# hank-kuo-cs/Volumetric-Primitives-Net

Measured on NVIDIA B200. Metric: primitive-loss fwd+bwd samples/sec, higher is better.
Workload: dtype f32

## Files before the change

### volumetric-primitives-net_b200/csrc/chamfer_tc.cu

```cuda
#include <cuda_fp16.h>
#include "common.cuh"

namespace vpn {

constexpr int kTcBlk = 128;
constexpr int kTcEpiWarps = 16;
constexpr int kTcThreads = (kTcEpiWarps + 4) * 32;
constexpr int kTcBlkBytes = kTcBlk * 32;
constexpr float kTcBig = 1.0e30f;
constexpr int kTcDefaultHunits = 0;

__device__ __forceinline__ uint32_t tc_smem_u32(const void* p) { return (uint32_t)__cvta_generic_to_shared(p); }
__device__ __forceinline__ float tc_inf() { return __int_as_float(0x7f800000); }

__device__ __forceinline__ uint64_t tc_desc(uint32_t saddr) {
  return (uint64_t)((saddr & 0x3FFFF) >> 4) | ((uint64_t)(128 >> 4) << 16) | ((uint64_t)(256 >> 4) << 32) | (1ull << 46);
}
constexpr uint32_t kTcIdesc = (1u << 4) | (0u << 7) | (0u << 10) | ((uint32_t)(2 * kTcBlk >> 3) << 17) | ((uint32_t)(kTcBlk >> 4) << 24);

constexpr uint32_t kTcIdescHalf = (1u << 4) | (0u << 7) | (0u << 10) | ((uint32_t)(kTcBlk >> 3) << 17) | ((uint32_t)(kTcBlk >> 4) << 24);
constexpr uint32_t kTcIdescHalfF16 = (0u << 4) | (0u << 7) | (0u << 10) | ((uint32_t)(kTcBlk >> 3) << 17) | ((uint32_t)(kTcBlk >> 4) << 24);

__device__ __forceinline__ void tc_mma(uint32_t d_tmem, uint64_t a, uint64_t b, uint32_t accumulate, uint32_t idesc = kTcIdesc) {
#if defined(VPN_TC_VARIANT) && VPN_TC_VARIANT == 3
// ... 85 lines not shown
  if (is_row) { x *= -2.f; y *= -2.f; z *= -2.f; }
  uint32_t hxy, lxy, hzn, lzn;
  tc_split2(x, y, hxy, lxy); tc_split2(z, n2, hzn, lzn);
  const uint32_t ones = 0x3c003c00u;
  uint4 k0, k1;
  if (is_row) {
    k0 = make_uint4(__byte_perm(hxy, hxy, 0x1010), __byte_perm(lxy, lxy, 0x1010), __byte_perm(hxy, hxy, 0x3232), __byte_perm(lxy, lxy, 0x3232));
    k1 = make_uint4(__byte_perm(hzn, hzn, 0x1010), __byte_perm(lzn, lzn, 0x1010), __byte_perm(hzn, lzn, 0x7632), ones);
  } else {
    const uint32_t wx = __byte_perm(hxy, lxy, 0x5410), wy = __byte_perm(hxy, lxy, 0x7632), wz = __byte_perm(hzn, lzn, 0x5410);
    k0 = make_uint4(wx, wx, wy, wy);
    k1 = make_uint4(wz, wz, ones, __byte_perm(hzn, lzn, 0x7632));
  }
  unsigned char* base = tile + (idx >> 3) * 256 + (idx & 7) * 16;
  *reinterpret_cast<uint4*>(base) = k0;
  *reinterpret_cast<uint4*>(base + 128) = k1;
  return n2;
}

struct TcSmem {
  unsigned char* rows; unsigned char* cols; float* rs_best; uint4* rs_mask; float* colw;
  u64* bars; float* red; uint32_t* tmem_slot; uint32_t* skip;
};
constexpr int kTcPlanWords = 128;
constexpr int kTcSkipWords = 128;
__host__ __device__ inline size_t tc_smem_bytes(int NB) {
  return (size_t)NB * kTcBlkBytes + 4 * kTcBlkBytes + 2 * (size_t)NB * kTcBlk * 20 + 2 * 2 * 2 * kTcBlk * 16 + 16 * 8 + 96 * 4 + 16 +
         kTcSkipWords * 4;
}
__device__ __forceinline__ TcSmem tc_carve(unsigned char* p, int NB) {
  TcSmem s;
  s.rows = p; p += (size_t)NB * kTcBlkBytes;
  s.cols = p; p += 4 * kTcBlkBytes;
  s.rs_best = reinterpret_cast<float*>(p); p += 2 * (size_t)NB * kTcBlk * 4;
  s.rs_mask = reinterpret_cast<uint4*>(p); p += 2 * (size_t)NB * kTcBlk * 16;
  s.colw = reinterpret_cast<float*>(p); p += 2 * 2 * 2 * kTcBlk * 16;
  s.bars = reinterpret_cast<u64*>(p); p += 16 * 8;
  s.red = reinterpret_cast<float*>(p); p += 96 * 4;
  s.tmem_slot = reinterpret_cast<uint32_t*>(p); p += 16;
  s.skip = reinterpret_cast<uint32_t*>(p);
  return s;
}

__device__ __forceinline__ float tc_lane_min4x32(uint32_t taddr, uint32_t empty_bar, int lane, float (&u)[4]) {
#if defined(VPN_TC_VARIANT) && VPN_TC_VARIANT == 2
  __syncwarp();
  if (lane == 0) tc_mbar_arrive(empty_bar);
// ... 274 lines not shown
  const float slack_rel = 6.103515625e-05f + 1.0986328125e-03f;
  const float slack_abs = __fmaf_ru(2.5025e-4f, rho2 * (S * S), 1.1930e-06f);
  if (tid == 0 && split == 0) tslack[(size_t)b * ntiles + tile_i] = make_float2(slack_rel, slack_abs * invS2);
  const uint32_t tbase = *sm.tmem_slot;

  const int nc = c_last - c_first;
  const int hc = (nc + 1) >> 1;
  const uint32_t* rawR = sm.skip; const uint32_t* rawC = sm.skip + 64;
  for (int i = tid; i < kTcPlanWords; i += kTcThreads) sm.skip[i] = plan_masks ? plan_masks[(size_t)cta * kTcPlanWords + i] : 0u;
  __syncthreads();
  if (warp == kTcEpiWarps + 2 && stats != nullptr) {
    unsigned s0 = 0, s1 = 0;
    for (int c = lane; c < nc; c += 32) { s0 += __popc(rawR[c] & ((1u << NB) - 1u)); s1 += __popc(rawC[c] & ((1u << NB) - 1u)); }
#pragma unroll
    for (int o = 16; o > 0; o >>= 1) { s0 += __shfl_xor_sync(0xffffffffu, s0, o); s1 += __shfl_xor_sync(0xffffffffu, s1, o); }
    if (lane == 0) {
      atomicAdd(&stats[0], (u64)(2 * nc * NB));
      atomicAdd(&stats[1], (u64)(s0 + s1));
#ifdef VPN_TC_COUNTERS
      atomicAdd(&stats[6], (u64)(nc * NB - s0));
      atomicAdd(&stats[7], (u64)(nc * NB - s1));
#endif
    }
  }
#ifdef VPN_TC_COUNTERS
  long long t_mark = 0;
  if (tid == 0 && stats != nullptr) {
    unsigned livechunks = 0, passes = 0;
    for (int c = 0; c < nc; ++c) livechunks += ((~rawC[c]) & ((1u << NB) - 1u)) ? 1u : 0u;
    for (int cc = 0; cc < 2 * hc; ++cc) passes += tc_pass_needed(cc < hc ? cc : cc - hc, nc, NB, cc < hc ? rawR : rawC) ? 1u : 0u;
    atomicAdd(&stats[8], (u64)livechunks);
    atomicAdd(&stats[9], (u64)passes);
    t_mark = clock64();
    atomicAdd(&stats[2], (u64)(t_mark - t_start));
  }
#define TC_MARK(slot) if (tid == 0 && stats != nullptr) { const long long t_ = clock64(); atomicAdd(&stats[slot], (u64)(t_ - t_mark)); t_mark = t_; }
#else
#define TC_MARK(slot)
#endif
  if (warp >= kTcEpiWarps && warp < kTcEpiWarps + 2) {
    const int g = warp - kTcEpiWarps;
    uint32_t seq = 0;
    float tx[4], ty[4], tz[4];
    const uint32_t nbmask = (1u << NB) - 1u;
    auto next_needed = [&](int cc) { while (cc < 2 * hc && !tc_pass_needed(cc < hc ? cc : cc - hc, nc, NB, cc < hc ? rawR : rawC)) ++cc; return cc; };
    auto half_live = [&](int cc) {
// ... 99 lines not shown
      for (uint32_t live = ~rawR[2 * j + h] & nbmask & (0x55555555u << p); live; live &= live - 1) {
        const int r = __ffs((int)live) - 1;
        tc_mbar_wait(my_full, it & 1);
        tc_fence_after();
        float mu[4];
        const float m = tc_lane_min4x32_h<HUNITS>(tlane, my_empty, lane, mu);
        ++it;
        const int ri = r * kTcBlk + li;
        const float best = my_best[ri];
        if (m <= tc_thr(best, slack_rel, slack_abs)) {
          const float t = tc_thr(fminf(best, m), slack_rel, slack_abs);
          const uint32_t nib = (mu[0] <= t ? 1u : 0u) | (mu[1] <= t ? 2u : 0u) | (mu[2] <= t ? 4u : 0u) | (mu[3] <= t ? 8u : 0u);
          if (tc_thr(m, slack_rel, slack_abs) < best) my_mask[ri] = make_uint4(0u, 0u, 0u, 0u);
          reinterpret_cast<uint32_t*>(my_mask + ri)[j >> 3] |= nib << ((j & 7) * 4);
          if (m < best) my_best[ri] = m;
        }
      }
    }
    TC_MARK(3)
    int cseq = 0;
    float4* xch = reinterpret_cast<float4*>(sm.colw) + (size_t)p * 4 * kTcBlk;
    for (int c = p; c < nc; c += 2) {
      const uint32_t livec = ~rawC[c] & nbmask;
      if (livec == 0u) {
        const int col = (c_first + c) * kTcBlk + li;
        if (h == 0 && col < M) { const size_t o = ((size_t)b * ntiles + tile_i) * M + col; cbest[o] = tc_inf(); cmask[o] = 0ull; }
        continue;
      }
      float best = tc_inf(); u64 mask = 0ull;
      for (uint32_t live = livec & (0x55555555u << h); live; live &= live - 1) {
        const int r = __ffs((int)live) - 1;
        tc_mbar_wait(my_full, it & 1);
        tc_fence_after();
        float mu[4];
        const float m = tc_lane_min4x32_h<HUNITS>(tlane, my_empty, lane, mu);
        ++it;
        if (m <= tc_thr(best, slack_rel, slack_abs)) {
          const float t = tc_thr(fminf(best, m), slack_rel, slack_abs);
          const uint32_t nib = (mu[0] <= t ? 1u : 0u) | (mu[1] <= t ? 2u : 0u) | (mu[2] <= t ? 4u : 0u) | (mu[3] <= t ? 8u : 0u);
          const float tm = tc_thr(m, slack_rel, slack_abs);
          mask = ((tm < best) ? 0ull : mask) | ((u64)nib << (4 * r));
          best = fminf(best, m);
        }
      }
      float4* slot = xch + (size_t)(cseq & 1) * 2 * kTcBlk;
      slot[h * kTcBlk + li] = make_float4(best, __uint_as_float((uint32_t)mask), __uint_as_float((uint32_t)(mask >> 32)), 0.f);
      asm volatile("bar.sync %0, 64;" :: "r"(1 + q + 4 * p) : "memory");
      if ((cseq & 1) == h) {
        const int col = (c_first + c) * kTcBlk + li;
        if (col < M) {
          const float4 other = slot[(h ^ 1) * kTcBlk + li];
// ... 3 lines not shown
          const u64 m2 = ((best <= t) ? mask : 0ull) | ((other.x <= t) ? omask : 0ull);
          const size_t o = ((size_t)b * ntiles + tile_i) * M + col;
          cbest[o] = b2 * invS2; cmask[o] = m2;
        }
      }
      ++cseq;
    }
  }
  TC_MARK(4)
  tc_fence_before();
  __syncthreads();
  if (warp == 0) asm volatile("tcgen05.dealloc.cta_group::1.sync.aligned.b32 %0, 512;" :: "r"(tbase) : "memory");
  const size_t mask_plane = (size_t)gridDim.x / ntiles * P;
  for (int i = tid; i < TM; i += kTcThreads) {
    const int row = tile_i * TM + i;
    if (row < P) {
      const float b0 = sm.rs_best[i], b1 = sm.rs_best[TM + i];
      const float best = fminf(b0, b1);
      const float t = tc_thr(best, slack_rel, slack_abs);
      const uint4 k0 = sm.rs_mask[i], k1 = sm.rs_mask[TM + i];
      const bool in0 = b0 <= t, in1 = b1 <= t;
      const size_t o = ((size_t)b * nsplit + split) * P + row;
      rbest[o] = best * invS2;
      rmask[o] = (in0 ? tc_spread_nibbles(k0.x) : 0ull) | (in1 ? (tc_spread_nibbles(k1.x) << 4) : 0ull);
      rmask[mask_plane + o] = (in0 ? tc_spread_nibbles(k0.y) : 0ull) | (in1 ? (tc_spread_nibbles(k1.y) << 4) : 0ull);
      rmask[2 * mask_plane + o] = (in0 ? tc_spread_nibbles(k0.z) : 0ull) | (in1 ? (tc_spread_nibbles(k1.z) << 4) : 0ull);
      rmask[3 * mask_plane + o] = (in0 ? tc_spread_nibbles(k0.w) : 0ull) | (in1 ? (tc_spread_nibbles(k1.w) << 4) : 0ull);
    }
  }
  TC_MARK(5)
}

__global__ void __launch_bounds__(256)
chamfer_flagged_kernel(const float* __restrict__ p1, const float* __restrict__ p2, float* __restrict__ min1,
                       int* __restrict__ idx1, float* __restrict__ min2, int* __restrict__ idx2,
                       const int* __restrict__ fallback, int P, int M) {
  const int b = blockIdx.y;
  if (fallback[b] == 0) return;
  const float* A = p1 + (size_t)b * P * 3;
  const float* T = p2 + (size_t)b * M * 3;
  for (int dir = 0; dir < 2; ++dir) {
    const float* X = dir ? T : A; const float* Y = dir ? A : T;
    const int nx = dir ? M : P, ny = dir ? P : M;
    float* mn = (dir ? min2 + (size_t)b * M : min1 + (size_t)b * P);
    int* ix = (dir ? idx2 + (size_t)b * M : idx1 + (size_t)b * P);
    for (int i = blockIdx.x * blockDim.x + threadIdx.x; i < nx; i += gridDim.x * blockDim.x) {
      const float x = X[3 * (size_t)i], y = X[3 * (size_t)i + 1], z = X[3 * (size_t)i + 2];
      float bv = tc_inf(); int bj = 0;
      bool nan_seen = false;
      for (int j = 0; j < ny; ++j) {
// ... 9 lines not shown
  }
}

__global__ void __launch_bounds__(256)
chamfer_tc_bounds_kernel(const float* __restrict__ p2, float* __restrict__ tmax, int M) {
  __shared__ float red[8];
  const float* T = p2 + (size_t)blockIdx.x * M * 3;
  float m = 0.f;
  for (int i = threadIdx.x; i < 3 * M; i += 256) {
    const float v = fabsf(T[i]);
    m = (v <= m) ? m : v;
  }
#pragma unroll
  for (int o = 16; o > 0; o >>= 1) { const float x = __shfl_xor_sync(0xffffffffu, m, o); m = (x <= m) ? m : x; }
  if ((threadIdx.x & 31) == 0) red[threadIdx.x >> 5] = m;
  __syncthreads();
  if (threadIdx.x == 0) {
    for (int w = 1; w < 8; ++w) m = (red[w] <= m) ? m : red[w];
    tmax[blockIdx.x] = m;
  }
}

size_t chamfer_tc_smem_bytes(int NB) { return tc_smem_bytes(NB); }
int chamfer_tc_plan_words() { return kTcPlanWords; }


int chamfer_tc_launch(const float* p1, const float* p2, float* rbest, u64* rmask, float* cbest, u64* cmask,
                      float2* tslack, int* fallback, float* tmax, const float* cbox, const float* rbox, const float* rthr,
                      const float* cub, u64* stats, uint32_t* plan_masks, int* plan_work, int* plan_order, int with_bounds,
                      int B, int P, int M, int NB, int ntiles, int nsplit, int nchunks, int cps, cudaStream_t s) {
  static DeviceOnce once;
  const size_t smem = tc_smem_bytes(NB);
  {
    cudaError_t e = set_dyn_smem(chamfer_tc_kernel<0>, (int)tc_smem_bytes(16), once);
    for (int k = 0; k < 4 && e == cudaSuccess; ++k) {
      void (*kern)(const float*, const float*, float*, u64*, float*, u64*, float2*, int*, const float*, const uint32_t*, const int*, u64*,
                   int, int, int, int, int, int, int) = k == 0 ? chamfer_tc_kernel<1> : (k == 1 ? chamfer_tc_kernel<2> : (k == 2 ? chamfer_tc_kernel<3> : chamfer_tc_kernel<4>));
      static DeviceOnce more[4];
      e = set_dyn_smem(kern, (int)tc_smem_bytes(16), more[k]);
    }
    if (e != cudaSuccess) { vpn_set_error("chamfer tc: smem attribute: %s", cudaGetErrorString(e)); return VPN_ERR_CUDA; }
  }
  int rc;
  if (with_bounds) {
    chamfer_tc_bounds_kernel<<<B, 256, 0, s>>>(p2, tmax, M);
    if ((rc = vpn_check_launch("chamfer_tc_bounds_kernel"))) return rc;
  }
// ... 34 lines not shown
```

### volumetric-primitives-net_b200/csrc/chamfer_tiled.cu

```cuda
#include <cstdlib>
#include <mutex>
#include <type_traits>
#include "common.cuh"

namespace vpn {

enum { MODE_EXACT = 0, MODE_DIFF = 1, MODE_EXPAND = 2, MODE_TC = 3 };

constexpr int kTThreads = 256;
constexpr int kTWarps = kTThreads / 32;
constexpr int kCW = 128;
constexpr int kMaxChunksPerSplit = 64;
constexpr float kBig = 1.0e30f;

__device__ __forceinline__ u64 pk(float a, float b) { u64 r; asm("mov.b64 %0, {%1,%2};" : "=l"(r) : "f"(a), "f"(b)); return r; }
__device__ __forceinline__ void upk(u64 v, float& a, float& b) { asm("mov.b64 {%0,%1}, %2;" : "=f"(a), "=f"(b) : "l"(v)); }
__device__ __forceinline__ u64 add2(u64 a, u64 b) { u64 r; asm("add.rn.f32x2 %0, %1, %2;" : "=l"(r) : "l"(a), "l"(b)); return r; }
__device__ __forceinline__ u64 sub2(u64 a, u64 b) { u64 r; asm("sub.rn.f32x2 %0, %1, %2;" : "=l"(r) : "l"(a), "l"(b)); return r; }
__device__ __forceinline__ u64 mul2(u64 a, u64 b) { u64 r; asm("mul.rn.f32x2 %0, %1, %2;" : "=l"(r) : "l"(a), "l"(b)); return r; }
__device__ __forceinline__ u64 fma2(u64 a, u64 b, u64 c) { u64 r; asm("fma.rn.f32x2 %0, %1, %2, %3;" : "=l"(r) : "l"(a), "l"(b), "l"(c)); return r; }
__device__ __forceinline__ float min3f(float a, float b, float c) { float r; asm("min.f32 %0, %1, %2, %3;" : "=f"(r) : "f"(a), "f"(b), "f"(c)); return r; }
__device__ __forceinline__ float warp_min_f32(float a) { float r; asm volatile("redux.sync.min.f32 %0, %1, 0xffffffff;" : "=f"(r) : "f"(a)); return r; }
__device__ __forceinline__ float inf_f() { return __int_as_float(0x7f800000); }

// ... 457 lines not shown
              d[kk] = exact_d2s(rc.x, rc.y, rc.z, q.x, q.y, q.z);
              dm = fminf(dm, d[kk]);
            }
            int at;
            const int st = unit_scan(d, dm, lane, &at);
            if (st == 1) atomicMin(&key[r], ((u64)__float_as_uint(sqrtf(dm)) << 32) | (unsigned)__float_as_int(src[at].w));
            else if (st == 2) { const u64 kv = unit_exact_walk(rc.x, rc.y, rc.z, src, 0, 1); if (kv != ~0ull) atomicMin(&key[r], kv); }
          }
          group_sync(bar);
        }
        if (valid) {
          const u64 kv = key[gt];
          const size_t orow = orow_of();
          min1[orow] = __uint_as_float((unsigned)(kv >> 32));
          idx1[orow] = (int)(unsigned)(kv & 0xffffffffu);
        }
        group_sync(bar);
      }
    }
  }
}

__global__ void chamfer_col_thr_kernel(const float* __restrict__ cbest, const float2* __restrict__ tslack,
                                       float* __restrict__ cthr, int M, int ntiles) {
  const int b = blockIdx.y;
  const int col = blockIdx.x * blockDim.x + threadIdx.x;
  if (col >= M) return;
  float g = inf_f(), rel = 0.f, ab = 0.f;
  for (int ti = 0; ti < ntiles; ++ti) {
    g = fminf(g, cbest[((size_t)b * ntiles + ti) * M + col]);
    const float2 sl = tslack[(size_t)b * ntiles + ti];
    rel = fmaxf(rel, sl.x); ab = fmaxf(ab, sl.y);
  }
  cthr[(size_t)b * M + col] = thr_of(g, rel, ab);
}

template <int R, bool TC, int NT>
__global__ void __launch_bounds__(NT, 1024 / NT)
chamfer_recover_cols_kernel(const float* __restrict__ p1, const float* __restrict__ p2,
                            const float* __restrict__ cbest, const void* __restrict__ cmask_,
                            const float* __restrict__ cthr, u64* __restrict__ key2, int P, int M, int ntiles,
                            const int* __restrict__ skip, const int* __restrict__ rperm) {
  constexpr int TM = TC ? 128 * R : kTThreads * R;
  constexpr int kSub = TC ? 1 : ((R >= 4) ? 4 : R);
  constexpr int kRunsPerSub = TC ? 1 : R / kSub;
  constexpr int kPer = TC ? 4096 / NT : 8;
  constexpr int kBitBits = TC ? 6 : 4;
  using mask_t = typename std::conditional<TC, u64, unsigned>::type;
  const mask_t* __restrict__ cmask = reinterpret_cast<const mask_t*>(cmask_);
  const mask_t kBitMask = TC ? (mask_t)((4 * R >= 64) ? ~0ull : ((1ull << (4 * R)) - 1ull)) : (mask_t)0xffu;
  if (skip && skip[blockIdx.y]) return;
  extern __shared__ __align__(16) unsigned char smem_raw[];
  float4* rows = reinterpret_cast<float4*>(smem_raw);
  __shared__ unsigned items[kItemCap];
  __shared__ int warp_sums[33];
  const int b = blockIdx.y, ti = blockIdx.x, tid = threadIdx.x, lane = tid & 31;
  const float* A = p1 + (size_t)b * P * 3;
  const float qnan = __int_as_float(0x7fc00000);
  for (int i = tid; i < TM; i += NT) {
    int rowi = ti * TM + i;
    rows[i] = rowi < P ? make_float4(A[3 * (size_t)rowi], A[3 * (size_t)rowi + 1], A[3 * (size_t)rowi + 2],
                                     __int_as_float(rperm ? rperm[(size_t)b * P + rowi] : rowi))
                       : make_float4(qnan, qnan, qnan, __int_as_float(0x7fffffff));
  }
  const size_t rec0 = ((size_t)b * ntiles + ti) * M;
  for (int slab = 0; slab < M; slab += NT * kPer) {
    mask_t mk[kPer];
    int cnt = 0;
#pragma unroll
    for (int u = 0; u < kPer; ++u) {
      const int col = slab + u * NT + tid;
      mk[u] = 0;
      if (col < M && cbest[rec0 + col] <= cthr[(size_t)b * M + col]) mk[u] = cmask[rec0 + col] & kBitMask;
      cnt += TC ? __popcll((u64)mk[u]) : __popc((unsigned)mk[u]);
    }
    int total;
    const int off = block_exclusive_scan<NT>(cnt, warp_sums, &total);
    for (int base = 0; base < total; base += kItemCap) {
      int j = off;
#pragma unroll
      for (int u = 0; u < kPer; ++u)
        for (mask_t mm = mk[u]; mm; mm &= mm - 1, ++j)
          if (j >= base && j < base + kItemCap)
            items[j - base] = ((unsigned)(u * NT + tid) << kBitBits) |
                              (unsigned)((TC ? __ffsll((long long)mm) : __ffs((int)mm)) - 1);
      __syncthreads();
      const int units = min(kItemCap, total - base) * kSub;
      for (int it = tid; it < units; it += NT) {
        const unsigned item = items[it / kSub];
        const int col = slab + (int)(item >> kBitBits), w = item & ((1u << kBitBits) - 1u), sub = it % kSub;
        const float* t = p2 + 3 * ((size_t)b * M + col);
        const float tx = __ldg(t), ty = __ldg(t + 1), tz = __ldg(t + 2);
        u64 best = ~0ull;
#pragma unroll 1
        for (int rr = sub * kRunsPerSub; rr < (sub + 1) * kRunsPerSub; ++rr) {
          const int base_row = TC ? (w * 32) : (rr * kTThreads + w * 32);
// ... 13 lines not shown
        }
        if (best != ~0ull) atomicMin(&key2[(size_t)b * M + col], best);
      }
      __syncthreads();
    }
  }
}

__global__ void chamfer_unpack_key_kernel(const u64* __restrict__ key, float* __restrict__ mn, int* __restrict__ idx, size_t n,
                                          const int* __restrict__ skip, int per_sample, const int* __restrict__ perm) {
  size_t i = (size_t)blockIdx.x * blockDim.x + threadIdx.x;
  if (i >= n) return;
  const size_t smp = i / (size_t)per_sample;
  if (skip && skip[smp]) return;
  u64 k = key[i];
  const size_t o = perm ? smp * (size_t)per_sample + (size_t)perm[i] : i;
  mn[o] = __uint_as_float((unsigned)(k >> 32));
  idx[o] = (int)(unsigned)(k & 0xffffffffu);
}

struct TiledPlan { int R, ntiles, nchunks, nsplit, cps, tc, TM; };

size_t chamfer_tc_smem_bytes(int NB);
int chamfer_tc_plan_words();
int chamfer_tc_launch(const float* p1, const float* p2, float* rbest, u64* rmask, float* cbest, u64* cmask,
                      float2* tslack, int* fallback, float* tmax, const float* cbox, const float* rbox, const float* rthr,
                      const float* cub, u64* stats, unsigned* plan_masks, int* plan_work, int* plan_order, int with_bounds,
                      int B, int P, int M, int NB, int ntiles, int nsplit, int nchunks, int cps, cudaStream_t s);
int chamfer_prep_launch(const float* p1, const float* p2, float* p2s, float4* p2v, int* perm, float* cbox, float* rbox, float* rthr,
                        float* cub, float* tmax, float* p1s, int* rperm, unsigned long long* stats, int B, int P, int M, cudaStream_t s);
int chamfer_flagged_launch(const float* p1, const float* p2, float* min1, int* idx1, float* min2, int* idx2,
                           const int* fallback, int B, int P, int M, cudaStream_t s);

static void finish_plan(TiledPlan& pl, int B, long long slots, int min_cps) {
  long long base = (long long)pl.ntiles * B;
  long long s = (4 * slots + base - 1) / base;
  long long smin = (pl.nchunks + kMaxChunksPerSplit - 1) / kMaxChunksPerSplit;
  long long smax = pl.nchunks / min_cps;
  if (s > smax) s = smax;
  if (s < smin) s = smin;
  if (s > pl.nchunks) s = pl.nchunks;
  if (s < 1) s = 1;
  pl.cps = (int)((pl.nchunks + s - 1) / s);
  pl.nsplit = (pl.nchunks + pl.cps - 1) / pl.cps;
}

static bool make_plan(int B, int P, int M, int sm_count, TiledPlan& pl) {
// ... 42 lines not shown
struct TiledWs { size_t rbest, rmask, cbest, cmask, tslack, fallback, tmax, cthr, key2, p2s, p2v, perm, cbox, rbox, rthr, cub, pmask, pwork, porder, p1s, rperm, total; };
static TiledWs ws_layout(int B, int P, int M, const TiledPlan& pl) {
  TiledWs w; size_t o = 0;
  w.rbest = o; o += al256((size_t)B * pl.nsplit * P * 4);
  w.rmask = o; o += al256((size_t)B * pl.nsplit * P * 8 * (pl.tc ? 4 : 1));
  w.cbest = o; o += al256((size_t)B * pl.ntiles * M * 4);
  w.cmask = o; o += al256((size_t)B * pl.ntiles * M * (pl.tc ? 8 : 4));
  w.tslack = o; o += al256((size_t)B * pl.ntiles * 8);
  w.fallback = o; o += al256((size_t)B * 4 + 8 + 128);
  w.tmax = o; o += al256((size_t)B * 4);
  w.cthr = o; o += al256((size_t)B * M * 4);
  w.key2 = o; o += al256((size_t)B * M * 8);
  w.p2s = w.p2v = w.perm = w.cbox = w.rbox = w.rthr = w.cub = w.pmask = w.pwork = w.porder = w.p1s = w.rperm = 0;
  if (pl.tc) {
    const size_t nrb = (size_t)(P + 127) / 128;
    w.p2s = o; o += al256((size_t)B * M * 12);
    w.p2v = o; o += al256((size_t)B * pl.nchunks * kCW * 16);
    w.perm = o; o += al256((size_t)B * M * 4);
    w.cbox = o; o += al256((size_t)B * pl.nchunks * 32);
    w.rbox = o; o += al256((size_t)B * nrb * 32);
    w.rthr = o; o += al256((size_t)B * nrb * 4);
    w.cub = o; o += al256((size_t)B * pl.nchunks * 4);
    const size_t ncta = (size_t)pl.ntiles * pl.nsplit * B;
    w.pmask = o; o += al256(ncta * (size_t)chamfer_tc_plan_words() * 4);
    w.pwork = o; o += al256(ncta * 4);
    w.porder = o; o += al256(ncta * 4);
    w.p1s = o; o += al256((size_t)B * P * 12);
    w.rperm = o; o += al256((size_t)B * P * 4);
  }
  w.total = o;
  return w;
}

static bool plan_for(int mode, int B, int P, int M, TiledPlan& pl) {
  const int kPlanSms = device_sm_count();
  if (mode == MODE_TC) return make_plan_tc(B, P, M, kPlanSms, pl);
  if (mode >= 0) return make_plan(B, P, M, kPlanSms, pl);
  return make_plan_tc(B, P, M, kPlanSms, pl) || make_plan(B, P, M, kPlanSms, pl);
}

int chamfer_tiled_supported(int B, int P, int M, int mode) {
  TiledPlan pl;
  return plan_for(mode, B, P, M, pl) ? 1 : 0;
}

int chamfer_tiled_uses_tc(int B, int P, int M, int mode) {
  TiledPlan pl;
// ... 37 lines not shown
}

template <int R>
static int launch_main_mode(int mode, const float* p1, const float* p2, char* ws, const TiledWs& wl, const TiledPlan& pl,
                            int B, int P, int M, int only_flagged, cudaStream_t s) {
  switch (mode) {
    case MODE_EXACT: return launch_main<R, MODE_EXACT>(p1, p2, ws, wl, pl, B, P, M, only_flagged, s);
    case MODE_DIFF:  return launch_main<R, MODE_DIFF>(p1, p2, ws, wl, pl, B, P, M, only_flagged, s);
    default:         return launch_main<R, MODE_EXPAND>(p1, p2, ws, wl, pl, B, P, M, only_flagged, s);
  }
}

static int launch_any(int mode, const float* p1, const float* p2, char* ws, const TiledWs& wl, const TiledPlan& pl,
                      int B, int P, int M, int only_flagged, cudaStream_t s) {
  switch (pl.R) {
    case 16: return launch_main_mode<16>(mode, p1, p2, ws, wl, pl, B, P, M, only_flagged, s);
    case 8:  return launch_main_mode<8>(mode, p1, p2, ws, wl, pl, B, P, M, only_flagged, s);
    default: return launch_main_mode<4>(mode, p1, p2, ws, wl, pl, B, P, M, only_flagged, s);
  }
}

template <int R, bool TC>
static int launch_recover_cols(const float* p1, const float* p2, const float* cb, const void* cmk, const float* cthr,
                               u64* key2, int B, int P, int M, int ntiles, const int* skip, const int* rperm, cudaStream_t s) {
  static DeviceOnce once, once_half;
  const size_t smem = (size_t)(TC ? 128 * R : kTThreads * R) * sizeof(float4);
  if (TC && (long long)ntiles * B >= 2LL * device_sm_count()) {
    if (set_dyn_smem(chamfer_recover_cols_kernel<R, TC, 512>, (int)smem, once_half) != cudaSuccess) {
      vpn_set_error("chamfer tiled: smem attribute (cols recovery)"); return VPN_ERR_CUDA;
    }
    chamfer_recover_cols_kernel<R, TC, 512><<<dim3(ntiles, B), 512, smem, s>>>(p1, p2, cb, cmk, cthr, key2, P, M, ntiles, skip, rperm);
    return vpn_check_launch("chamfer_recover_cols_kernel");
  }
  if (set_dyn_smem(chamfer_recover_cols_kernel<R, TC, kRecThreads>, (int)smem, once) != cudaSuccess) {
    vpn_set_error("chamfer tiled: smem attribute (cols recovery)"); return VPN_ERR_CUDA;
  }
  chamfer_recover_cols_kernel<R, TC, kRecThreads><<<dim3(ntiles, B), kRecThreads, smem, s>>>(p1, p2, cb, cmk, cthr, key2, P, M, ntiles, skip, rperm);
  return vpn_check_launch("chamfer_recover_cols_kernel");
}

struct SideStream { cudaStream_t s = nullptr; cudaEvent_t fork = nullptr, join = nullptr; bool ok = false; std::mutex mu; };
static SideStream g_side[64];
static SideStream* side_stream_for(cudaStream_t s) {
  int dev = 0;
  if (cudaGetDevice(&dev) != cudaSuccess || dev < 0 || dev >= 64) return nullptr;
  SideStream& ss = g_side[dev];
  if (ss.ok) return &ss;
  cudaStreamCaptureStatus st = cudaStreamCaptureStatusNone;
  if (cudaStreamIsCapturing(s, &st) != cudaSuccess || st != cudaStreamCaptureStatusNone) { cudaGetLastError(); return nullptr; }
  std::lock_guard<std::mutex> lock(ss.mu);
  if (!ss.ok) {
    if (cudaStreamCreateWithFlags(&ss.s, cudaStreamNonBlocking) != cudaSuccess ||
        cudaEventCreateWithFlags(&ss.fork, cudaEventDisableTiming) != cudaSuccess ||
        cudaEventCreateWithFlags(&ss.join, cudaEventDisableTiming) != cudaSuccess) { cudaGetLastError(); return nullptr; }
    ss.ok = true;
  }
  return &ss;
}

int chamfer_tiled_fwd(const float* p1, const float* p2, float* min1, int* idx1, float* min2, int* idx2,
                      int B, int P, int M, void* ws_, size_t ws_bytes, int mode, cudaStream_t s, cudaEvent_t* ev) {
  TiledPlan pl;
  if (!plan_for(mode, B, P, M, pl)) { vpn_set_error("chamfer tiled: unsupported shape"); return VPN_ERR_SHAPE; }
  if (mode < 0) mode = pl.tc ? MODE_TC : MODE_EXPAND;
  TiledWs wl = ws_layout(B, P, M, pl);
  if (ws_bytes < wl.total) { vpn_set_error("chamfer tiled: workspace too small (%zu < %zu)", ws_bytes, wl.total); return VPN_ERR_WORKSPACE; }
  char* ws = reinterpret_cast<char*>(ws_);
  int* fallback = reinterpret_cast<int*>(ws + wl.fallback);
  const int* skip = nullptr;
  int rc;
  if (ev) cudaEventRecord(ev[0], s);
  const size_t flag_bytes = (((size_t)B * 4 + 7) & ~(size_t)7) + 128;
  if (mode == MODE_EXPAND || mode == MODE_TC) {
    if (cudaMemsetAsync(fallback, 0, flag_bytes, s) != cudaSuccess) { vpn_set_error("chamfer tiled: memset failed"); return VPN_ERR_CUDA; }
  }
  const float* p2w = p2;
  const int* perm = nullptr;
  const float4* p2v = nullptr;
  const float* p1w = p1;
  const int* rperm = nullptr;
  if (mode == MODE_TC) {
    float* p2s = reinterpret_cast<float*>(ws + wl.p2s);
    int* pm = reinterpret_cast<int*>(ws + wl.perm);
    float* cbox = reinterpret_cast<float*>(ws + wl.cbox); float* rbox = reinterpret_cast<float*>(ws + wl.rbox);
    float* rthr = reinterpret_cast<float*>(ws + wl.rthr); float* cub = reinterpret_cast<float*>(ws + wl.cub);
    float* tmax = reinterpret_cast<float*>(ws + wl.tmax);
    u64* stats = reinterpret_cast<u64*>(ws + wl.fallback + (((size_t)B * 4 + 7) & ~(size_t)7));
    const bool prune = tuning_value(kTuneTcPrune) != 2;
    if (prune) {
      float4* pv = reinterpret_cast<float4*>(ws + wl.p2v);
      float* p1s = reinterpret_cast<float*>(ws + wl.p1s);
      int* rp = reinterpret_cast<int*>(ws + wl.rperm);
      if ((rc = chamfer_prep_launch(p1, p2, p2s, pv, pm, cbox, rbox, rthr, cub, tmax, p1s, rp, stats, B, P, M, s))) return rc;
      p2w = p2s; perm = pm; p2v = pv; p1w = p1s; rperm = rp;
    }
    rc = chamfer_tc_launch(p1w, p2w, reinterpret_cast<float*>(ws + wl.rbest), reinterpret_cast<u64*>(ws + wl.rmask),
                           reinterpret_cast<float*>(ws + wl.cbest), reinterpret_cast<u64*>(ws + wl.cmask),
                           reinterpret_cast<float2*>(ws + wl.tslack), fallback, tmax, prune ? cbox : nullptr, rbox, rthr, cub, stats,
                           reinterpret_cast<unsigned*>(ws + wl.pmask), reinterpret_cast<int*>(ws + wl.pwork),
                           reinterpret_cast<int*>(ws + wl.porder), prune ? 0 : 1, B, P, M, pl.R, pl.ntiles, pl.nsplit, pl.nchunks,
                           pl.cps, s);
    if (rc) return rc;
    if (ev) cudaEventRecord(ev[1], s);
    if ((rc = chamfer_flagged_launch(p1, p2, min1, idx1, min2, idx2, fallback, B, P, M, s))) return rc;
    skip = fallback;
  } else {
    if ((rc = launch_any(mode, p1, p2, ws, wl, pl, B, P, M, 0, s))) return rc;
    if (ev) cudaEventRecord(ev[1], s);
    if (mode == MODE_EXPAND) {
      if ((rc = launch_any(MODE_DIFF, p1, p2, ws, wl, pl, B, P, M, 1, s))) return rc;
    }
  }
  if (ev) cudaEventRecord(ev[2], s);
  SideStream* side = tuning_value(kTuneSerialRecovery) ? nullptr : side_stream_for(s);
  std::unique_lock<std::mutex> side_lock;
  cudaStream_t sc = s;
  if (side) {
// ... 4 lines not shown
  {
    static DeviceOnce once_rows;
    const size_t smem_rows = kRowsFixedSmem + (size_t)(pl.nchunks < kSegChunks ? pl.nchunks : kSegChunks) * kCW * sizeof(float4);
    if (set_dyn_smem(chamfer_recover_rows_kernel, (int)(kRowsFixedSmem + kSegChunks * kCW * sizeof(float4)), once_rows) != cudaSuccess) {
      vpn_set_error("chamfer tiled: smem attribute (rows recovery)"); return VPN_ERR_CUDA;
    }
    const int nblk = (P + kRowGroup - 1) / kRowGroup;
    const long long nitems = (long long)nblk * B;
    if (nitems > 0x7fffffffLL) { vpn_set_error("chamfer tiled: too many row blocks"); return VPN_ERR_SHAPE; }
    const int sms = device_sm_count();
    chamfer_recover_rows_kernel<<<(unsigned)(nitems < sms ? nitems : sms), kRecThreads, smem_rows, s>>>(
        p1w, p2w, p2v, pl.nchunks * kCW, reinterpret_cast<const float*>(ws + wl.rbest), reinterpret_cast<const u64*>(ws + wl.rmask),
        pl.tc ? 4 : 1, (size_t)B * pl.nsplit * P, reinterpret_cast<const float2*>(ws + wl.tslack), min1, idx1, P, M, pl.nchunks,
        pl.nsplit, pl.cps, pl.TM, pl.ntiles, skip, nblk, (int)nitems, rperm);
    if ((rc = vpn_check_launch("chamfer_recover_rows_kernel"))) return rc;
  }
  if (ev) cudaEventRecord(ev[3], s);
  const float* cb = reinterpret_cast<const float*>(ws + wl.cbest);
  const void* cmk = ws + wl.cmask;
  const float2* tsl = reinterpret_cast<const float2*>(ws + wl.tslack);
  float* cthr = reinterpret_cast<float*>(ws + wl.cthr);
  u64* key2 = reinterpret_cast<u64*>(ws + wl.key2);
  if (cudaMemsetAsync(key2, 0xFF, (size_t)B * M * 8, sc) != cudaSuccess) { vpn_set_error("chamfer tiled: memset failed"); return VPN_ERR_CUDA; }
  chamfer_col_thr_kernel<<<dim3((M + 255) / 256, B), 256, 0, sc>>>(cb, tsl, cthr, M, pl.ntiles);
  if ((rc = vpn_check_launch("chamfer_col_thr_kernel"))) return rc;
  if (pl.tc) {
    switch (pl.R) {
      case 16: rc = launch_recover_cols<16, true>(p1w, p2w, cb, cmk, cthr, key2, B, P, M, pl.ntiles, skip, rperm, sc); break;
      case 8:  rc = launch_recover_cols<8, true>(p1w, p2w, cb, cmk, cthr, key2, B, P, M, pl.ntiles, skip, rperm, sc); break;
      default: rc = launch_recover_cols<4, true>(p1w, p2w, cb, cmk, cthr, key2, B, P, M, pl.ntiles, skip, rperm, sc); break;
    }
  } else {
    switch (pl.R) {
      case 16: rc = launch_recover_cols<16, false>(p1, p2, cb, cmk, cthr, key2, B, P, M, pl.ntiles, skip, nullptr, sc); break;
      case 8:  rc = launch_recover_cols<8, false>(p1, p2, cb, cmk, cthr, key2, B, P, M, pl.ntiles, skip, nullptr, sc); break;
      default: rc = launch_recover_cols<4, false>(p1, p2, cb, cmk, cthr, key2, B, P, M, pl.ntiles, skip, nullptr, sc); break;
    }
  }
  if (rc) return rc;
  {
    size_t n = (size_t)B * M;
    chamfer_unpack_key_kernel<<<(unsigned)((n + 255) / 256), 256, 0, sc>>>(key2, min2, idx2, n, skip, M, perm);
  }
  rc = vpn_check_launch("chamfer_unpack_key_kernel");
  if (side) {
    if (cudaEventRecord(side->join, sc) != cudaSuccess || cudaStreamWaitEvent(s, side->join, 0) != cudaSuccess) {
      vpn_set_error("chamfer tiled: stream join failed"); rc = VPN_ERR_CUDA;
    }
  }
  if (ev) cudaEventRecord(ev[4], s);
  return rc;
}

}
```

### volumetric-primitives-net_b200/csrc/common.cuh

```cuda
#pragma once
#include <cuda_runtime.h>
#include <stdint.h>
#include <atomic>

#define VPN_OK 0
#define VPN_ERR_CUDA (-1)
#define VPN_ERR_SHAPE (-2)
#define VPN_ERR_ARG (-3)
#define VPN_ERR_WORKSPACE (-4)

#define VPN_PI 3.1415927410125732f

void vpn_set_error(const char* fmt, ...);
int vpn_check_launch(const char* what);

namespace vpn {

typedef unsigned long long u64;

struct DeviceOnce { std::atomic<unsigned long long> mask{0}; };
template <typename K>
inline cudaError_t set_dyn_smem(K kernel, int bytes, DeviceOnce& once) {
  int dev = 0;
  cudaError_t e = cudaGetDevice(&dev);
  if (e != cudaSuccess) return e;
  const unsigned long long bit = dev < 64 ? (1ull << dev) : 0ull;
  if (bit && (once.mask.load(std::memory_order_acquire) & bit)) return cudaSuccess;
  e = cudaFuncSetAttribute(kernel, cudaFuncAttributeMaxDynamicSharedMemorySize, bytes);
  if (e == cudaSuccess && bit) once.mask.fetch_or(bit, std::memory_order_release);
  return e;
}
int device_sm_count();
int tuning_value(int key);
enum { kTuneTiledR = 0, kTuneTcNb = 1, kTuneEmdCluster = 2, kTuneTcPrune = 3, kTuneSerialRecovery = 4, kTuneArVariant = 5, kTuneArCtas = 6, kTuneArThreads = 7, kTuneArGridDiv = 8, kTunePrepNearCols = 9, kTunePrepRepsCols = 10, kTunePrepNearRows = 11, kTunePrepRepsRows = 12, kTunePrepProbe = 13, kTunePrepDeterministic = 14, kTuneTcHunits = 15, kTuneCount = 16 };

struct Pose {
  float r[9];
  float qn[4];
  float s, c;
  float len;
};

__device__ __forceinline__ float mod1(float w) {
  float m = fmodf(w, 1.0f);
  if (m != 0.0f && m < 0.0f) m += 1.0f;
  return m;
}

__device__ __forceinline__ void make_pose(const float* __restrict__ q, Pose& p) {
  float a = q[0], b = q[1], cc = q[2], w = q[3];
  float half = __fdiv_rn(__fmul_rn(__fmul_rn(mod1(w), 2.0f), VPN_PI), 2.0f);
  float s = sinf(half), c = cosf(half);
  float ux = a * s, uy = b * s, uz = cc * s, uw = c;
  float len = sqrtf(ux * ux + uy * uy + uz * uz + uw * uw);
  float x = ux / len, y = uy / len, z = uz / len, ww = uw / len;
  p.s = s; p.c = c; p.len = len;
  p.qn[0] = x; p.qn[1] = y; p.qn[2] = z; p.qn[3] = ww;
// ... 53 lines not shown
```

Baseline: 34500.

## Skip writing dead column records and consult prune plan in downstream col kernels

The tensor-core chamfer kernel no longer writes inf/zero sentinel records for fully pruned column chunks. Instead the column-threshold and column-recovery kernels read the prune plan masks and treat those records as dead, so the redundant stores and later reads are avoided. The col-threshold loop is restructured into 32-tile batches with a warp ballot over the plan words. It also adds counter-only diagnostics under a compile flag. The risk is that correctness now depends on the plan indexing in the two consumers matching exactly.

```diff
diff --git a/volumetric-primitives-net_b200/csrc/chamfer_tc.cu b/volumetric-primitives-net_b200/csrc/chamfer_tc.cu
--- a/volumetric-primitives-net_b200/csrc/chamfer_tc.cu
+++ b/volumetric-primitives-net_b200/csrc/chamfer_tc.cu
@@ -131,7 +131,6 @@
   unsigned char* rows; unsigned char* cols; float* rs_best; uint4* rs_mask; float* colw;
   u64* bars; float* red; uint32_t* tmem_slot; uint32_t* skip;
 };
-constexpr int kTcPlanWords = 128;
 constexpr int kTcSkipWords = 128;
 __host__ __device__ inline size_t tc_smem_bytes(int NB) {
   return (size_t)NB * kTcBlkBytes + 4 * kTcBlkBytes + 2 * (size_t)NB * kTcBlk * 20 + 2 * 2 * 2 * kTcBlk * 16 + 16 * 8 + 96 * 4 + 16 +
@@ -452,6 +451,13 @@
       atomicAdd(&stats[7], (u64)(nc * NB - s1));
 #endif
     }
+#ifdef VPN_TC_COUNTERS
+    unsigned sdead = 0;
+    for (int c = lane; c < nc; c += 32) sdead += (rawC[c] & ((1u << NB) - 1u)) == ((1u << NB) - 1u) ? 1u : 0u;
+#pragma unroll
+    for (int o = 16; o > 0; o >>= 1) sdead += __shfl_xor_sync(0xffffffffu, sdead, o);
+    if (lane == 0) atomicAdd(&stats[14], (u64)sdead | ((u64)nc << 32));
+#endif
   }
 #ifdef VPN_TC_COUNTERS
   long long t_mark = 0;
@@ -597,11 +603,7 @@
     float4* xch = reinterpret_cast<float4*>(sm.colw) + (size_t)p * 4 * kTcBlk;
     for (int c = p; c < nc; c += 2) {
       const uint32_t livec = ~rawC[c] & nbmask;
-      if (livec == 0u) {
-        const int col = (c_first + c) * kTcBlk + li;
-        if (h == 0 && col < M) { const size_t o = ((size_t)b * ntiles + tile_i) * M + col; cbest[o] = tc_inf(); cmask[o] = 0ull; }
-        continue;
-      }
+      if (livec == 0u) continue;
       float best = tc_inf(); u64 mask = 0ull;
       for (uint32_t live = livec & (0x55555555u << h); live; live &= live - 1) {
         const int r = __ffs((int)live) - 1;
@@ -651,10 +653,30 @@
       const bool in0 = b0 <= t, in1 = b1 <= t;
       const size_t o = ((size_t)b * nsplit + split) * P + row;
       rbest[o] = best * invS2;
-      rmask[o] = (in0 ? tc_spread_nibbles(k0.x) : 0ull) | (in1 ? (tc_spread_nibbles(k1.x) << 4) : 0ull);
-      rmask[mask_plane + o] = (in0 ? tc_spread_nibbles(k0.y) : 0ull) | (in1 ? (tc_spread_nibbles(k1.y) << 4) : 0ull);
-      rmask[2 * mask_plane + o] = (in0 ? tc_spread_nibbles(k0.z) : 0ull) | (in1 ? (tc_spread_nibbles(k1.z) << 4) : 0ull);
-      rmask[3 * mask_plane + o] = (in0 ? tc_spread_nibbles(k0.w) : 0ull) | (in1 ? (tc_spread_nibbles(k1.w) << 4) : 0ull);
+      const u64 w0 = (in0 ? tc_spread_nibbles(k0.x) : 0ull) | (in1 ? (tc_spread_nibbles(k1.x) << 4) : 0ull);
+      const u64 w1 = (in0 ? tc_spread_nibbles(k0.y) : 0ull) | (in1 ? (tc_spread_nibbles(k1.y) << 4) : 0ull);
+      const u64 w2 = (in0 ? tc_spread_nibbles(k0.z) : 0ull) | (in1 ? (tc_spread_nibbles(k1.z) << 4) : 0ull);
+      const u64 w3 = (in0 ? tc_spread_nibbles(k0.w) : 0ull) | (in1 ? (tc_spread_nibbles(k1.w) << 4) : 0ull);
+      rmask[o] = w0; rmask[mask_plane + o] = w1; rmask[2 * mask_plane + o] = w2; rmask[3 * mask_plane + o] = w3;
+#ifdef VPN_TC_COUNTERS
+      if (stats != nullptr) {
+        const unsigned grp = __activemask();
+        const int n = __popcll(w0) + __popcll(w1) + __popcll(w2) + __popcll(w3);
+        const u64 x0 = __shfl_xor_sync(grp, w0, 1), x1 = __shfl_xor_sync(grp, w1, 1), x2 = __shfl_xor_sync(grp, w2, 1), x3 = __shfl_xor_sync(grp, w3, 1);
+        const bool has_pair = (grp >> (lane ^ 1)) & 1u;
+        const bool shared = has_pair && ((w0 & x0) | (w1 & x1) | (w2 & x2) | (w3 & x3)) != 0ull;
+        const unsigned pr = __ballot_sync(grp, (lane & 1) == 0 && has_pair), sh = __ballot_sync(grp, (lane & 1) == 0 && shared);
+        u64 add[3];
+#pragma unroll
+        for (int k = 0; k < 3; ++k)
+          add[k] = (u64)__popc(__ballot_sync(grp, n == 2 * k)) | ((u64)__popc(__ballot_sync(grp, k == 2 ? n >= 5 : n == 2 * k + 1)) << 32);
+        if (lane == __ffs(grp) - 1) {
+#pragma unroll
+          for (int k = 0; k < 3; ++k) atomicAdd(&stats[10 + k], add[k]);
+          atomicAdd(&stats[13], (u64)__popc(sh) | ((u64)__popc(pr) << 32));
+        }
+      }
+#endif
     }
   }
   TC_MARK(5)
@@ -710,7 +732,6 @@
 }
 
 size_t chamfer_tc_smem_bytes(int NB) { return tc_smem_bytes(NB); }
-int chamfer_tc_plan_words() { return kTcPlanWords; }
 
 
 int chamfer_tc_launch(const float* p1, const float* p2, float* rbest, u64* rmask, float* cbest, u64* cmask,
diff --git a/volumetric-primitives-net_b200/csrc/chamfer_tiled.cu b/volumetric-primitives-net_b200/csrc/chamfer_tiled.cu
--- a/volumetric-primitives-net_b200/csrc/chamfer_tiled.cu
+++ b/volumetric-primitives-net_b200/csrc/chamfer_tiled.cu
@@ -503,17 +503,26 @@
 }
 
 __global__ void chamfer_col_thr_kernel(const float* __restrict__ cbest, const float2* __restrict__ tslack,
-                                       float* __restrict__ cthr, int M, int ntiles) {
-  const int b = blockIdx.y;
+                                       float* __restrict__ cthr, int M, int ntiles,
+                                       const uint32_t* __restrict__ plan, int nsplit, int cps, uint32_t nbmask) {
+  const int b = blockIdx.y, lane = threadIdx.x & 31;
   const int col = blockIdx.x * blockDim.x + threadIdx.x;
-  if (col >= M) return;
+  const int chunk = min(col, M - 1) / kCW;
   float g = inf_f(), rel = 0.f, ab = 0.f;
-  for (int ti = 0; ti < ntiles; ++ti) {
-    g = fminf(g, cbest[((size_t)b * ntiles + ti) * M + col]);
-    const float2 sl = tslack[(size_t)b * ntiles + ti];
-    rel = fmaxf(rel, sl.x); ab = fmaxf(ab, sl.y);
-  }
-  cthr[(size_t)b * M + col] = thr_of(g, rel, ab);
+  for (int t0 = 0; t0 < ntiles; t0 += 32) {
+    const uint32_t dead = plan ? __ballot_sync(0xffffffffu, t0 + lane < ntiles &&
+                                               tc_col_record_pruned(plan, b, t0 + lane, chunk, ntiles, nsplit, cps, nbmask)) : 0u;
+    const int n = min(32, ntiles - t0);
+#pragma unroll 8
+    for (int j = 0; j < n; ++j) {
+      const int ti = t0 + j;
+      const float v = (col < M && !((dead >> j) & 1u)) ? cbest[((size_t)b * ntiles + ti) * M + col] : inf_f();
+      g = fminf(g, v);
+      const float2 sl = tslack[(size_t)b * ntiles + ti];
+      rel = fmaxf(rel, sl.x); ab = fmaxf(ab, sl.y);
+    }
+  }
+  if (col < M) cthr[(size_t)b * M + col] = thr_of(g, rel, ab);
 }
 
 template <int R, bool TC, int NT>
@@ -521,12 +530,14 @@
 chamfer_recover_cols_kernel(const float* __restrict__ p1, const float* __restrict__ p2,
                             const float* __restrict__ cbest, const void* __restrict__ cmask_,
                             const float* __restrict__ cthr, u64* __restrict__ key2, int P, int M, int ntiles,
-                            const int* __restrict__ skip, const int* __restrict__ rperm) {
+                            const int* __restrict__ skip, const int* __restrict__ rperm,
+                            const uint32_t* __restrict__ plan, int nsplit, int cps) {
   constexpr int TM = TC ? 128 * R : kTThreads * R;
   constexpr int kSub = TC ? 1 : ((R >= 4) ? 4 : R);
   constexpr int kRunsPerSub = TC ? 1 : R / kSub;
   constexpr int kPer = TC ? 4096 / NT : 8;
   constexpr int kBitBits = TC ? 6 : 4;
+  static_assert(!TC || NT * kPer == 32 * kCW, "a slab of the tensor-core records spans 32 chunks");
   using mask_t = typename std::conditional<TC, u64, unsigned>::type;
   const mask_t* __restrict__ cmask = reinterpret_cast<const mask_t*>(cmask_);
   const mask_t kBitMask = TC ? (mask_t)((4 * R >= 64) ? ~0ull : ((1ull << (4 * R)) - 1ull)) : (mask_t)0xffu;
@@ -546,13 +557,19 @@
   }
   const size_t rec0 = ((size_t)b * ntiles + ti) * M;
   for (int slab = 0; slab < M; slab += NT * kPer) {
+    uint32_t dead = 0u;
+    if (TC && plan) {
+      const int ch = slab / kCW + lane;
+      dead = __ballot_sync(0xffffffffu, ch * kCW < M && tc_col_record_pruned(plan, b, ti, ch, ntiles, nsplit, cps, (uint32_t)((1ull << R) - 1ull)));
+    }
     mask_t mk[kPer];
     int cnt = 0;
 #pragma unroll
     for (int u = 0; u < kPer; ++u) {
       const int col = slab + u * NT + tid;
       mk[u] = 0;
-      if (col < M && cbest[rec0 + col] <= cthr[(size_t)b * M + col]) mk[u] = cmask[rec0 + col] & kBitMask;
+      if (col < M && !(TC && ((dead >> ((col - slab) / kCW)) & 1u)) && cbest[rec0 + col] <= cthr[(size_t)b * M + col])
+        mk[u] = cmask[rec0 + col] & kBitMask;
       cnt += TC ? __popcll((u64)mk[u]) : __popc((unsigned)mk[u]);
     }
     int total;
@@ -612,7 +629,6 @@
 struct TiledPlan { int R, ntiles, nchunks, nsplit, cps, tc, TM; };
 
 size_t chamfer_tc_smem_bytes(int NB);
-int chamfer_tc_plan_words();
 int chamfer_tc_launch(const float* p1, const float* p2, float* rbest, u64* rmask, float* cbest, u64* cmask,
                       float2* tslack, int* fallback, float* tmax, const float* cbox, const float* rbox, const float* rthr,
                       const float* cub, u64* stats, unsigned* plan_masks, int* plan_work, int* plan_order, int with_bounds,
@@ -701,7 +717,7 @@
     w.rthr = o; o += al256((size_t)B * nrb * 4);
     w.cub = o; o += al256((size_t)B * pl.nchunks * 4);
     const size_t ncta = (size_t)pl.ntiles * pl.nsplit * B;
-    w.pmask = o; o += al256(ncta * (size_t)chamfer_tc_plan_words() * 4);
+    w.pmask = o; o += al256(ncta * (size_t)kTcPlanWords * 4);
     w.pwork = o; o += al256(ncta * 4);
     w.porder = o; o += al256(ncta * 4);
     w.p1s = o; o += al256((size_t)B * P * 12);
@@ -785,20 +801,21 @@
 
 template <int R, bool TC>
 static int launch_recover_cols(const float* p1, const float* p2, const float* cb, const void* cmk, const float* cthr,
-                               u64* key2, int B, int P, int M, int ntiles, const int* skip, const int* rperm, cudaStream_t s) {
+                               u64* key2, int B, int P, int M, int ntiles, const int* skip, const int* rperm,
+                               const uint32_t* plan, int nsplit, int cps, cudaStream_t s) {
   static DeviceOnce once, once_half;
   const size_t smem = (size_t)(TC ? 128 * R : kTThreads * R) * sizeof(float4);
   if (TC && (long long)ntiles * B >= 2LL * device_sm_count()) {
     if (set_dyn_smem(chamfer_recover_cols_kernel<R, TC, 512>, (int)smem, once_half) != cudaSuccess) {
       vpn_set_error("chamfer tiled: smem attribute (cols recovery)"); return VPN_ERR_CUDA;
     }
-    chamfer_recover_cols_kernel<R, TC, 512><<<dim3(ntiles, B), 512, smem, s>>>(p1, p2, cb, cmk, cthr, key2, P, M, ntiles, skip, rperm);
+    chamfer_recover_cols_kernel<R, TC, 512><<<dim3(ntiles, B), 512, smem, s>>>(p1, p2, cb, cmk, cthr, key2, P, M, ntiles, skip, rperm, plan, nsplit, cps);
     return vpn_check_launch("chamfer_recover_cols_kernel");
   }
   if (set_dyn_smem(chamfer_recover_cols_kernel<R, TC, kRecThreads>, (int)smem, once) != cudaSuccess) {
     vpn_set_error("chamfer tiled: smem attribute (cols recovery)"); return VPN_ERR_CUDA;
   }
-  chamfer_recover_cols_kernel<R, TC, kRecThreads><<<dim3(ntiles, B), kRecThreads, smem, s>>>(p1, p2, cb, cmk, cthr, key2, P, M, ntiles, skip, rperm);
+  chamfer_recover_cols_kernel<R, TC, kRecThreads><<<dim3(ntiles, B), kRecThreads, smem, s>>>(p1, p2, cb, cmk, cthr, key2, P, M, ntiles, skip, rperm, plan, nsplit, cps);
   return vpn_check_launch("chamfer_recover_cols_kernel");
 }
 
@@ -842,6 +859,7 @@
   const float4* p2v = nullptr;
   const float* p1w = p1;
   const int* rperm = nullptr;
+  const uint32_t* plan = nullptr;
   if (mode == MODE_TC) {
     float* p2s = reinterpret_cast<float*>(ws + wl.p2s);
     int* pm = reinterpret_cast<int*>(ws + wl.perm);
@@ -855,7 +873,7 @@
       float* p1s = reinterpret_cast<float*>(ws + wl.p1s);
       int* rp = reinterpret_cast<int*>(ws + wl.rperm);
       if ((rc = chamfer_prep_launch(p1, p2, p2s, pv, pm, cbox, rbox, rthr, cub, tmax, p1s, rp, stats, B, P, M, s))) return rc;
-      p2w = p2s; perm = pm; p2v = pv; p1w = p1s; rperm = rp;
+      p2w = p2s; perm = pm; p2v = pv; p1w = p1s; rperm = rp; plan = reinterpret_cast<const uint32_t*>(ws + wl.pmask);
     }
     rc = chamfer_tc_launch(p1w, p2w, reinterpret_cast<float*>(ws + wl.rbest), reinterpret_cast<u64*>(ws + wl.rmask),
                            reinterpret_cast<float*>(ws + wl.cbest), reinterpret_cast<u64*>(ws + wl.cmask),
@@ -906,19 +924,20 @@
   float* cthr = reinterpret_cast<float*>(ws + wl.cthr);
   u64* key2 = reinterpret_cast<u64*>(ws + wl.key2);
   if (cudaMemsetAsync(key2, 0xFF, (size_t)B * M * 8, sc) != cudaSuccess) { vpn_set_error("chamfer tiled: memset failed"); return VPN_ERR_CUDA; }
-  chamfer_col_thr_kernel<<<dim3((M + 255) / 256, B), 256, 0, sc>>>(cb, tsl, cthr, M, pl.ntiles);
+  chamfer_col_thr_kernel<<<dim3((M + 255) / 256, B), 256, 0, sc>>>(cb, tsl, cthr, M, pl.ntiles, plan, pl.nsplit, pl.cps,
+                                                                     (uint32_t)((1ull << pl.R) - 1ull));
   if ((rc = vpn_check_launch("chamfer_col_thr_kernel"))) return rc;
   if (pl.tc) {
     switch (pl.R) {
-      case 16: rc = launch_recover_cols<16, true>(p1w, p2w, cb, cmk, cthr, key2, B, P, M, pl.ntiles, skip, rperm, sc); break;
-      case 8:  rc = launch_recover_cols<8, true>(p1w, p2w, cb, cmk, cthr, key2, B, P, M, pl.ntiles, skip, rperm, sc); break;
-      default: rc = launch_recover_cols<4, true>(p1w, p2w, cb, cmk, cthr, key2, B, P, M, pl.ntiles, skip, rperm, sc); break;
+      case 16: rc = launch_recover_cols<16, true>(p1w, p2w, cb, cmk, cthr, key2, B, P, M, pl.ntiles, skip, rperm, plan, pl.nsplit, pl.cps, sc); break;
+      case 8:  rc = launch_recover_cols<8, true>(p1w, p2w, cb, cmk, cthr, key2, B, P, M, pl.ntiles, skip, rperm, plan, pl.nsplit, pl.cps, sc); break;
+      default: rc = launch_recover_cols<4, true>(p1w, p2w, cb, cmk, cthr, key2, B, P, M, pl.ntiles, skip, rperm, plan, pl.nsplit, pl.cps, sc); break;
     }
   } else {
     switch (pl.R) {
-      case 16: rc = launch_recover_cols<16, false>(p1, p2, cb, cmk, cthr, key2, B, P, M, pl.ntiles, skip, nullptr, sc); break;
-      case 8:  rc = launch_recover_cols<8, false>(p1, p2, cb, cmk, cthr, key2, B, P, M, pl.ntiles, skip, nullptr, sc); break;
-      default: rc = launch_recover_cols<4, false>(p1, p2, cb, cmk, cthr, key2, B, P, M, pl.ntiles, skip, nullptr, sc); break;
+      case 16: rc = launch_recover_cols<16, false>(p1, p2, cb, cmk, cthr, key2, B, P, M, pl.ntiles, skip, nullptr, nullptr, 1, 1, sc); break;
+      case 8:  rc = launch_recover_cols<8, false>(p1, p2, cb, cmk, cthr, key2, B, P, M, pl.ntiles, skip, nullptr, nullptr, 1, 1, sc); break;
+      default: rc = launch_recover_cols<4, false>(p1, p2, cb, cmk, cthr, key2, B, P, M, pl.ntiles, skip, nullptr, nullptr, 1, 1, sc); break;
     }
   }
   if (rc) return rc;
diff --git a/volumetric-primitives-net_b200/csrc/common.cuh b/volumetric-primitives-net_b200/csrc/common.cuh
--- a/volumetric-primitives-net_b200/csrc/common.cuh
+++ b/volumetric-primitives-net_b200/csrc/common.cuh
@@ -33,6 +33,14 @@
 int device_sm_count();
 int tuning_value(int key);
 enum { kTuneTiledR = 0, kTuneTcNb = 1, kTuneEmdCluster = 2, kTuneTcPrune = 3, kTuneSerialRecovery = 4, kTuneArVariant = 5, kTuneArCtas = 6, kTuneArThreads = 7, kTuneArGridDiv = 8, kTunePrepNearCols = 9, kTunePrepRepsCols = 10, kTunePrepNearRows = 11, kTunePrepRepsRows = 12, kTunePrepProbe = 13, kTunePrepDeterministic = 14, kTuneTcHunits = 15, kTuneCount = 16 };
+
+constexpr int kTcPlanWords = 128;
+__device__ __forceinline__ bool tc_col_record_pruned(const uint32_t* __restrict__ plan, int b, int ti, int chunk, int ntiles,
+                                                     int nsplit, int cps, uint32_t nbmask) {
+  const int s = chunk / cps;
+  const uint32_t w = __ldg(plan + ((size_t)((size_t)b * nsplit + s) * ntiles + ti) * kTcPlanWords + 64 + (chunk - s * cps));
+  return (w & nbmask) == nbmask;
+}
 
 struct Pose {
   float r[9];
```

Result: no change. 34780, median of 6 (+0.8%).
